# OpenNLPLab/ACR_WSSS

Measured on NVIDIA B200. Metric: train_imgs_per_sec, higher is better.
Workload: dtype bf16

## Files before the change

acr_wsss_b200/csrc/gelu.cu:

```cuda
#include "common.cuh"
#include <cuda_bf16.h>

namespace {

constexpr float kRsqrt2 = 0.70710678118654752440f;
constexpr float kRsqrt2Pi = 0.39894228040143267794f;
constexpr int kGeluChunks = 64;

__device__ __forceinline__ void phi_and_exp(float x, float& phi, float& e) {
  const float ax = fabsf(x);
  float t;
  asm("rcp.approx.ftz.f32 %0, %1;" : "=f"(t) : "f"(fmaf(0.3275911f * kRsqrt2, ax, 1.f)));
  asm("ex2.approx.ftz.f32 %0, %1;" : "=f"(e) : "f"(x * x * -0.72134752044448170368f));
  float p = 0.5f * 1.061405429f;
  p = fmaf(p, t, 0.5f * -1.453152027f);
  p = fmaf(p, t, 0.5f * 1.421413741f);
  p = fmaf(p, t, 0.5f * -0.284496736f);
  p = fmaf(p, t, 0.5f * 0.254829592f);
  const float h = p * t * e;
  phi = x < 0.f ? h : 1.f - h;
}
__device__ __forceinline__ float gelu_f(float x) {
  float phi, e;
  phi_and_exp(x, phi, e);
  return x * phi;
}
__device__ __forceinline__ float gelu_grad_f(float x) {
  float phi, e;
  phi_and_exp(x, phi, e);
  return fmaf(x * kRsqrt2Pi, e, phi);
}

__device__ __forceinline__ void unpack8(const uint4& v, float* f) {
  const __nv_bfloat162* h = reinterpret_cast<const __nv_bfloat162*>(&v);
#pragma unroll
  for (int i = 0; i < 4; ++i) {
    const float2 t = __bfloat1622float2(h[i]);
    f[2 * i] = t.x;
    f[2 * i + 1] = t.y;
  }
}
__device__ __forceinline__ uint4 pack8(const float* f) {
  uint4 v;
  __nv_bfloat162* h = reinterpret_cast<__nv_bfloat162*>(&v);
#pragma unroll
  for (int i = 0; i < 4; ++i) h[i] = __floats2bfloat162_rn(f[2 * i], f[2 * i + 1]);
  return v;
}

__global__ void __launch_bounds__(256)
gelu_fwd_kernel(const __nv_bfloat16* __restrict__ x, __nv_bfloat16* __restrict__ y, long long n) {
  const long long nv = n >> 3;
  const long long stride = (long long)gridDim.x * blockDim.x;
  for (long long i = (long long)blockIdx.x * blockDim.x + threadIdx.x; i < nv; i += stride) {
    const uint4 v = __ldg(reinterpret_cast<const uint4*>(x) + i);
    float f[8];
    unpack8(v, f);
#pragma unroll
    for (int e = 0; e < 8; ++e) f[e] = gelu_f(f[e]);
    reinterpret_cast<uint4*>(y)[i] = pack8(f);
  }
  if (blockIdx.x == 0 && threadIdx.x < (n & 7)) {
    const long long i = (nv << 3) + threadIdx.x;
    y[i] = __float2bfloat16(gelu_f(__bfloat162float(x[i])));
  }
}

__global__ void __launch_bounds__(256)
gelu_bwd_kernel(const __nv_bfloat16* __restrict__ x, const __nv_bfloat16* __restrict__ dy, __nv_bfloat16* __restrict__ dx,
                int M, int F, int rows_per_chunk, float* __restrict__ partial) {
  __shared__ float red[8][32][9];
  const int cg = threadIdx.x & 31, ty = threadIdx.x >> 5;
  const int c = blockIdx.x * 256 + cg * 8;
  const int r0 = blockIdx.y * rows_per_chunk;
  const int r1 = min(M, r0 + rows_per_chunk);
  float acc[8];
#pragma unroll
  for (int e = 0; e < 8; ++e) acc[e] = 0.f;
  if (c < F) {
#pragma unroll 2
    for (int r = r0 + ty; r < r1; r += 8) {
      const size_t off = ((size_t)r * F + c) >> 3;
      const uint4 xv = __ldg(reinterpret_cast<const uint4*>(x) + off);
      const uint4 gv = __ldg(reinterpret_cast<const uint4*>(dy) + off);
      float xf[8], gf[8];
      unpack8(xv, xf);
      unpack8(gv, gf);
#pragma unroll
      for (int e = 0; e < 8; ++e) gf[e] *= gelu_grad_f(xf[e]);
      const uint4 o = pack8(gf);
      reinterpret_cast<uint4*>(dx)[off] = o;
      unpack8(o, gf);
#pragma unroll
      for (int e = 0; e < 8; ++e) acc[e] += gf[e];
    }
  }
  if (partial == nullptr) return;
#pragma unroll
  for (int e = 0; e < 8; ++e) red[ty][cg][e] = acc[e];
  __syncthreads();
  const int col = threadIdx.x;
  if (blockIdx.x * 256 + col < F) {
    float t = 0.f;
#pragma unroll
    for (int k = 0; k < 8; ++k) t += red[k][col >> 3][col & 7];
    partial[(size_t)blockIdx.y * F + blockIdx.x * 256 + col] = t;
  }
}

__global__ void __launch_bounds__(256)
gelu_colsum_finish_kernel(const float* __restrict__ partial, int nparts, int F, float* __restrict__ out, int accumulate) {
  __shared__ float red[4][64];
  const int cl = threadIdx.x & 63, grp = threadIdx.x >> 6;
  const int c = blockIdx.x * 64 + cl;
  float s0 = 0.f, s1 = 0.f;
  if (c < F) {
    int p = grp;
    for (; p + 4 < nparts; p += 8) {
      s0 += __ldg(partial + (size_t)p * F + c);
      s1 += __ldg(partial + (size_t)(p + 4) * F + c);
    }
    for (; p < nparts; p += 4) s0 += __ldg(partial + (size_t)p * F + c);
  }
  red[grp][cl] = s0 + s1;
  __syncthreads();
  if (grp == 0 && c < F) {
    const float s = (red[0][cl] + red[1][cl]) + (red[2][cl] + red[3][cl]);
    out[c] = accumulate ? out[c] + s : s;
  }
}

}

extern "C" int acr_gelu_fwd_bf16(const void* x, void* y, long long n, void* stream) {
  ACR_REQUIRE(x && y, ACR_E_INVAL, "acr_gelu_fwd_bf16: null pointer");
  ACR_REQUIRE(n > 0, ACR_E_INVAL, "acr_gelu_fwd_bf16: n must be positive");
  ACR_REQUIRE((((uintptr_t)x | (uintptr_t)y) & 15) == 0, ACR_E_ALIGN, "acr_gelu_fwd_bf16: 16-byte alignment required");
  const long long nv = (n + 7) >> 3;
  const unsigned grid = (unsigned)std::min<long long>((nv + 255) / 256, 148LL * 32);
  gelu_fwd_kernel<<<grid, 256, 0, (cudaStream_t)stream>>>((const __nv_bfloat16*)x, (__nv_bfloat16*)y, n);
  return acr::check_launch("gelu_fwd_kernel");
}

extern "C" size_t acr_gelu_bwd_workspace(int F) { return F > 0 ? (size_t)kGeluChunks * F * sizeof(float) : 0; }

extern "C" int acr_gelu_bwd_bf16(const void* x, const void* dy, void* dx, int M, int F, float* colsum, int accumulate,
                                 void* workspace, size_t workspace_bytes, void* stream) {
  ACR_REQUIRE(x && dy && dx, ACR_E_INVAL, "acr_gelu_bwd_bf16: null pointer");
  ACR_REQUIRE(M > 0 && F > 0 && F % 8 == 0, ACR_E_INVAL, "acr_gelu_bwd_bf16: F must be a positive multiple of 8");
  ACR_REQUIRE((((uintptr_t)x | (uintptr_t)dy | (uintptr_t)dx) & 15) == 0, ACR_E_ALIGN, "acr_gelu_bwd_bf16: 16-byte alignment required");
  ACR_REQUIRE(colsum == nullptr || (workspace != nullptr && workspace_bytes >= acr_gelu_bwd_workspace(F)), ACR_E_NOMEM,
              "acr_gelu_bwd_bf16: workspace too small");
  cudaStream_t st = (cudaStream_t)stream;
  const int chunks = M < kGeluChunks * 8 ? 1 : kGeluChunks;
  const int rows_per_chunk = (M + chunks - 1) / chunks;
  dim3 grid((F + 255) / 256, chunks);
  gelu_bwd_kernel<<<grid, 256, 0, st>>>((const __nv_bfloat16*)x, (const __nv_bfloat16*)dy, (__nv_bfloat16*)dx, M, F, rows_per_chunk,
                                        colsum ? (float*)workspace : nullptr);
  if (int e = acr::check_launch("gelu_bwd_kernel")) return e;
  if (colsum) {
    gelu_colsum_finish_kernel<<<(F + 63) / 64, 256, 0, st>>>((const float*)workspace, chunks, F, colsum, accumulate);
    return acr::check_launch("gelu_colsum_finish_kernel");
  }
  return 0;
}
```

acr_wsss_b200/csrc/layernorm.cu:

```cuda
#include "attn_tc.cuh"
#include <cuda_bf16.h>

namespace {

constexpr int kWarpsPerCta = 8;

template <bool BF16>
__device__ __forceinline__ float4 load4(const void* __restrict__ base, long long idx4) {
  if (BF16) {
    const uint2 u = __ldg(reinterpret_cast<const uint2*>(base) + idx4);
    const float2 a = __bfloat1622float2(*reinterpret_cast<const __nv_bfloat162*>(&u.x));
    const float2 b = __bfloat1622float2(*reinterpret_cast<const __nv_bfloat162*>(&u.y));
    return make_float4(a.x, a.y, b.x, b.y);
  }
  return __ldg(reinterpret_cast<const float4*>(base) + idx4);
}
template <bool BF16>
__device__ __forceinline__ void store4(void* __restrict__ base, long long idx4, float4 v) {
  if (BF16) {
    __nv_bfloat162 p0 = __floats2bfloat162_rn(v.x, v.y), p1 = __floats2bfloat162_rn(v.z, v.w);
    uint2 u;
    u.x = *reinterpret_cast<uint32_t*>(&p0);
    u.y = *reinterpret_cast<uint32_t*>(&p1);
    reinterpret_cast<uint2*>(base)[idx4] = u;
  } else {
    reinterpret_cast<float4*>(base)[idx4] = v;
  }
}

template <int VEC, bool OUT_BF16, bool X_BF16>
__global__ void __launch_bounds__(kWarpsPerCta * 32)
layernorm_fwd_kernel(const void* __restrict__ x, const void* __restrict__ res, void* __restrict__ sum_out, const float* __restrict__ gamma,
                     const float* __restrict__ beta, int M, float eps, void* __restrict__ y, float* __restrict__ mean, float* __restrict__ rstd) {
  constexpr int E = 128 * VEC;
  const int lane = threadIdx.x & 31;
  for (long long row = (long long)blockIdx.x * kWarpsPerCta + (threadIdx.x >> 5); row < M; row += (long long)gridDim.x * kWarpsPerCta) {
  float4 v[VEC];
  float s = 0.f;
#pragma unroll
  for (int i = 0; i < VEC; ++i) {
    v[i] = load4<X_BF16>(x, row * (E / 4) + i * 32 + lane);
    if (res != nullptr) {
      const float4 r = load4<X_BF16>(res, row * (E / 4) + i * 32 + lane);
      v[i] = make_float4(v[i].x + r.x, v[i].y + r.y, v[i].z + r.z, v[i].w + r.w);
      if (X_BF16) {
        v[i].x = __bfloat162float(__float2bfloat16(v[i].x)); v[i].y = __bfloat162float(__float2bfloat16(v[i].y));
        v[i].z = __bfloat162float(__float2bfloat16(v[i].z)); v[i].w = __bfloat162float(__float2bfloat16(v[i].w));
      }
      store4<X_BF16>(sum_out, row * (E / 4) + i * 32 + lane, v[i]);
    }
    s += (v[i].x + v[i].y) + (v[i].z + v[i].w);
  }
  const float mu = acr::warp_sum(s) * (1.f / E);
  float ss = 0.f;
#pragma unroll
  for (int i = 0; i < VEC; ++i) {
    const float a = v[i].x - mu, b = v[i].y - mu, c = v[i].z - mu, d = v[i].w - mu;
    ss += (a * a + b * b) + (c * c + d * d);
  }
  const float rs = rsqrtf(acr::warp_sum(ss) * (1.f / E) + eps);
  if (lane == 0) { mean[row] = mu; rstd[row] = rs; }
#pragma unroll
  for (int i = 0; i < VEC; ++i) {
    const float4 g = __ldg(reinterpret_cast<const float4*>(gamma) + i * 32 + lane);
    const float4 bb = __ldg(reinterpret_cast<const float4*>(beta) + i * 32 + lane);
    const float o0 = (v[i].x - mu) * rs * g.x + bb.x, o1 = (v[i].y - mu) * rs * g.y + bb.y;
    const float o2 = (v[i].z - mu) * rs * g.z + bb.z, o3 = (v[i].w - mu) * rs * g.w + bb.w;
    store4<OUT_BF16>(y, row * (E / 4) + i * 32 + lane, make_float4(o0, o1, o2, o3));
  }
  }
}

template <int VEC, bool DY_BF16, bool X_BF16, bool COLSUM = false>
__global__ void __launch_bounds__(kWarpsPerCta * 32)
layernorm_bwd_kernel(const void* __restrict__ dy, const void* __restrict__ dres, const void* __restrict__ x, const float* __restrict__ mean,
                     const float* __restrict__ rstd, const float* __restrict__ gamma, int M, int rows_per_cta,
                     void* __restrict__ dx, float* __restrict__ part_g, float* __restrict__ part_b, float* __restrict__ part_c) {
  constexpr int E = 128 * VEC;
  constexpr int NARR = COLSUM ? 3 : 2;
  extern __shared__ float4 acc_sm[];
  const int lane = threadIdx.x & 31, warp = threadIdx.x >> 5;
  float4* ag = acc_sm + (0 * kWarpsPerCta + warp) * (VEC * 32) + lane;
  float4* ab = acc_sm + (1 * kWarpsPerCta + warp) * (VEC * 32) + lane;
  float4* ac = acc_sm + ((COLSUM ? 2 : 1) * kWarpsPerCta + warp) * (VEC * 32) + lane;
  float4 g[VEC];
#pragma unroll
  for (int i = 0; i < VEC; ++i) {
    g[i] = __ldg(reinterpret_cast<const float4*>(gamma) + i * 32 + lane);
    ag[i * 32] = make_float4(0.f, 0.f, 0.f, 0.f);
    ab[i * 32] = make_float4(0.f, 0.f, 0.f, 0.f);
    if (COLSUM) ac[i * 32] = make_float4(0.f, 0.f, 0.f, 0.f);
  }
  const long long r0 = (long long)blockIdx.x * rows_per_cta;
  const long long r1 = min((long long)M, r0 + rows_per_cta);
  for (long long row = r0 + warp; row < r1; row += kWarpsPerCta) {
    const float mu = __ldg(mean + row), rs = __ldg(rstd + row);
    float4 d[VEC], xh[VEC];
    float s1 = 0.f, s2 = 0.f;
#pragma unroll
    for (int i = 0; i < VEC; ++i) {
      d[i] = load4<DY_BF16>(dy, row * (E / 4) + i * 32 + lane);
      const float4 xv = load4<X_BF16>(x, row * (E / 4) + i * 32 + lane);
      xh[i] = make_float4((xv.x - mu) * rs, (xv.y - mu) * rs, (xv.z - mu) * rs, (xv.w - mu) * rs);
    }
#pragma unroll
    for (int i = 0; i < VEC; ++i) {
      float4 tb = ab[i * 32], tg = ag[i * 32];
      tb.x += d[i].x; tb.y += d[i].y; tb.z += d[i].z; tb.w += d[i].w;
      tg.x += d[i].x * xh[i].x; tg.y += d[i].y * xh[i].y; tg.z += d[i].z * xh[i].z; tg.w += d[i].w * xh[i].w;
      ab[i * 32] = tb;
      ag[i * 32] = tg;
      d[i].x *= g[i].x; d[i].y *= g[i].y; d[i].z *= g[i].z; d[i].w *= g[i].w;
      s1 += (d[i].x + d[i].y) + (d[i].z + d[i].w);
      s2 += (d[i].x * xh[i].x + d[i].y * xh[i].y) + (d[i].z * xh[i].z + d[i].w * xh[i].w);
    }
    s1 = acr::warp_sum(s1) * (1.f / E);
    s2 = acr::warp_sum(s2) * (1.f / E);
#pragma unroll
    for (int i = 0; i < VEC; ++i) {
      float4 o;
      o.x = rs * (d[i].x - s1 - xh[i].x * s2); o.y = rs * (d[i].y - s1 - xh[i].y * s2);
      o.z = rs * (d[i].z - s1 - xh[i].z * s2); o.w = rs * (d[i].w - s1 - xh[i].w * s2);
      if (dres != nullptr) {
        const float4 r = load4<X_BF16>(dres, row * (E / 4) + i * 32 + lane);
        o.x += r.x; o.y += r.y; o.z += r.z; o.w += r.w;
      }
      store4<X_BF16>(dx, row * (E / 4) + i * 32 + lane, o);
      if (COLSUM) {
        if (X_BF16) {
          o.x = __bfloat162float(__float2bfloat16(o.x)); o.y = __bfloat162float(__float2bfloat16(o.y));
          o.z = __bfloat162float(__float2bfloat16(o.z)); o.w = __bfloat162float(__float2bfloat16(o.w));
        }
        float4 tc_ = ac[i * 32];
        tc_.x += o.x; tc_.y += o.y; tc_.z += o.z; tc_.w += o.w;
        ac[i * 32] = tc_;
      }
    }
  }
  __syncthreads();
  const float* accf = reinterpret_cast<const float*>(acc_sm);
  for (int a = 0; a < NARR; ++a) {
    float* dst = (a == 0 ? part_g : (a == 1 ? part_b : part_c)) + (long long)blockIdx.x * E;
    for (int c = threadIdx.x; c < E; c += kWarpsPerCta * 32) {
      float t = 0.f;
#pragma unroll
      for (int w = 0; w < kWarpsPerCta; ++w) t += accf[(a * kWarpsPerCta + w) * E + c];
      dst[c] = t;
    }
  }
}

__global__ void __launch_bounds__(1024)
layernorm_bwd_finish_kernel(const float* __restrict__ part_g, const float* __restrict__ part_b, const float* __restrict__ part_c, int nparts,
                            int E, float* __restrict__ dgamma, float* __restrict__ dbeta, float* __restrict__ dx_colsum, int accumulate) {
  __shared__ float sg[128][9], sb[128][9], sc[128][9];
  const int cl = threadIdx.x & 7, grp = threadIdx.x >> 3;
  const int c = blockIdx.x * 8 + cl;
  float ag = 0.f, ab = 0.f, ac = 0.f;
  if (c < E) {
#pragma unroll 3
    for (int p = grp; p < nparts; p += 128) {
      ag += __ldg(part_g + (long long)p * E + c);
      ab += __ldg(part_b + (long long)p * E + c);
      if (part_c != nullptr) ac += __ldg(part_c + (long long)p * E + c);
    }
  }
  sg[grp][cl] = ag;
  sb[grp][cl] = ab;
  sc[grp][cl] = ac;
  __syncthreads();
  if (threadIdx.x < 24 && blockIdx.x * 8 + (threadIdx.x & 7) < E) {
    const int arr = threadIdx.x >> 3, col = threadIdx.x & 7;
    const float (*src)[9] = arr == 0 ? sg : (arr == 1 ? sb : sc);
    float t0 = 0.f, t1 = 0.f, t2 = 0.f, t3 = 0.f;
#pragma unroll 8
    for (int k = 0; k < 128; k += 4) { t0 += src[k][col]; t1 += src[k + 1][col]; t2 += src[k + 2][col]; t3 += src[k + 3][col]; }
    const float t = (t0 + t1) + (t2 + t3);
    const int cc = blockIdx.x * 8 + col;
    if (arr == 0) dgamma[cc] = accumulate ? dgamma[cc] + t : t;
    else if (arr == 1) dbeta[cc] = accumulate ? dbeta[cc] + t : t;
    else if (dx_colsum != nullptr) dx_colsum[cc] = accumulate ? dx_colsum[cc] + t : t;
  }
}

constexpr int kColsumChunks = 64;

__global__ void __launch_bounds__(256)
colsum_bf16_kernel(const __nv_bfloat16* __restrict__ x, int M, int F, int rows_per_chunk, float* __restrict__ partial) {
  __shared__ float2 red[8][33];
  const int cp = threadIdx.x & 31, grp = threadIdx.x >> 5;
  const int c = blockIdx.x * 64 + cp * 2;
  const int r0 = blockIdx.y * rows_per_chunk;
  const int r1 = min(M, r0 + rows_per_chunk);
  float2 acc = make_float2(0.f, 0.f);
  if (c < F) {
    for (int r = r0 + grp; r < r1; r += 8) {
      const float2 v = __bfloat1622float2(*reinterpret_cast<const __nv_bfloat162*>(x + (size_t)r * F + c));
      acc.x += v.x;
      acc.y += v.y;
    }
  }
  red[grp][cp] = acc;
  __syncthreads();
  if (grp == 0 && c < F) {
    float2 t = make_float2(0.f, 0.f);
#pragma unroll
    for (int k = 0; k < 8; ++k) { t.x += red[k][cp].x; t.y += red[k][cp].y; }
    *reinterpret_cast<float2*>(partial + (size_t)blockIdx.y * F + c) = t;
  }
}

__global__ void __launch_bounds__(256)
colsum_finish_kernel(const float* __restrict__ partial, int nparts, int F, float* __restrict__ out, int accumulate) {
  __shared__ float red[4][64];
  const int cl = threadIdx.x & 63, grp = threadIdx.x >> 6;
  const int c = blockIdx.x * 64 + cl;
  float s0 = 0.f, s1 = 0.f;
  if (c < F) {
    int p = grp;
    for (; p + 4 < nparts; p += 8) {
      s0 += __ldg(partial + (size_t)p * F + c);
      s1 += __ldg(partial + (size_t)(p + 4) * F + c);
    }
    for (; p < nparts; p += 4) s0 += __ldg(partial + (size_t)p * F + c);
  }
  red[grp][cl] = s0 + s1;
  __syncthreads();
  if (grp == 0 && c < F) {
    const float s = (red[0][cl] + red[1][cl]) + (red[2][cl] + red[3][cl]);
    out[c] = accumulate ? out[c] + s : s;
  }
}

constexpr int kBwdCtas = 296;

template <int VEC>
int launch_fwd(const void* x, int x_bf16, const void* res, void* sum_out, const float* gamma, const float* beta, int M, float eps, void* y, int y_bf16, float* mean,
               float* rstd, cudaStream_t st) {
  const unsigned grid = (unsigned)std::min((M + kWarpsPerCta - 1) / kWarpsPerCta, 148 * 8);
  const int T = kWarpsPerCta * 32;
  if (x_bf16) {
    if (y_bf16) layernorm_fwd_kernel<VEC, true, true><<<grid, T, 0, st>>>(x, res, sum_out, gamma, beta, M, eps, y, mean, rstd);
    else layernorm_fwd_kernel<VEC, false, true><<<grid, T, 0, st>>>(x, res, sum_out, gamma, beta, M, eps, y, mean, rstd);
  } else {
    if (y_bf16) layernorm_fwd_kernel<VEC, true, false><<<grid, T, 0, st>>>(x, res, sum_out, gamma, beta, M, eps, y, mean, rstd);
    else layernorm_fwd_kernel<VEC, false, false><<<grid, T, 0, st>>>(x, res, sum_out, gamma, beta, M, eps, y, mean, rstd);
  }
  return acr::check_launch("layernorm_fwd_kernel");
}
template <int VEC>
int launch_bwd(const void* dy, int dy_bf16, const void* dres, const void* x, int x_bf16, const float* mean, const float* rstd, const float* gamma, int M,
               void* dx, float* dgamma, float* dbeta, float* dx_colsum, int accumulate, float* parts, cudaStream_t st) {
  constexpr int E = 128 * VEC;
  const int ctas = M < kBwdCtas * kWarpsPerCta ? (M + kWarpsPerCta - 1) / kWarpsPerCta : kBwdCtas;
  const int rows_per_cta = (M + ctas - 1) / ctas;
  float* pg = parts;
  float* pb = parts + (size_t)kBwdCtas * E;
  float* pc = dx_colsum ? parts + (size_t)2 * kBwdCtas * E : nullptr;
  const int T = kWarpsPerCta * 32;
#define ACR_LN_BWD(DYB, XB, CS)                                                                                              \
  do {                                                                                                                      \
    auto kfn = layernorm_bwd_kernel<VEC, DYB, XB, CS>;                                                                      \
    const size_t smem = (size_t)(CS ? 3 : 2) * kWarpsPerCta * E * sizeof(float);                                            \
    static bool attr_set[64] = {false};             \
    if (int e_ = acr_attn::set_max_smem(kfn, smem, attr_set)) return e_;                                                    \
    kfn<<<ctas, T, smem, st>>>(dy, dres, x, mean, rstd, gamma, M, rows_per_cta, dx, pg, pb, pc);                            \
  } while (0)
  if (pc != nullptr) {
    ACR_REQUIRE(x_bf16 && dy_bf16, ACR_E_INVAL, "acr_layernorm_bwd: dx_colsum needs bf16 x and dy");
    ACR_LN_BWD(true, true, true);
  } else if (x_bf16) {
    if (dy_bf16) ACR_LN_BWD(true, true, false);
    else ACR_LN_BWD(false, true, false);
  } else {
    if (dy_bf16) ACR_LN_BWD(true, false, false);
    else ACR_LN_BWD(false, false, false);
  }
#undef ACR_LN_BWD
  if (int e = acr::check_launch("layernorm_bwd_kernel")) return e;
  layernorm_bwd_finish_kernel<<<(E + 7) / 8, 1024, 0, st>>>(pg, pb, pc, ctas, E, dgamma, dbeta, dx_colsum, accumulate);
  return acr::check_launch("layernorm_bwd_finish_kernel");
}

}

extern "C" size_t acr_layernorm_bwd_workspace(int E) { return E > 0 ? (size_t)3 * kBwdCtas * E * sizeof(float) : 0; }

extern "C" int acr_layernorm_fwd(const void* x, int x_is_bf16, const void* residual, void* sum_out, const float* gamma, const float* beta,
                                 int M, int E, float eps, void* y, int y_is_bf16, float* mean, float* rstd, void* stream) {
  ACR_REQUIRE(x && gamma && beta && y && mean && rstd, ACR_E_INVAL, "acr_layernorm_fwd: null pointer");
  ACR_REQUIRE(M > 0 && E > 0 && E % 128 == 0 && E <= 2048, ACR_E_INVAL, "acr_layernorm_fwd: E=%d must be a multiple of 128, <= 2048", E);
  ACR_REQUIRE((residual == nullptr) == (sum_out == nullptr), ACR_E_INVAL, "acr_layernorm_fwd: residual and sum_out go together");
  ACR_REQUIRE((((uintptr_t)x | (uintptr_t)y | (uintptr_t)gamma | (uintptr_t)beta | (uintptr_t)residual | (uintptr_t)sum_out) & 15) == 0, ACR_E_ALIGN,
              "acr_layernorm_fwd: 16-byte alignment required");
  cudaStream_t st = (cudaStream_t)stream;
  switch (E / 128) {
    case 1: return launch_fwd<1>(x, x_is_bf16, residual, sum_out, gamma, beta, M, eps, y, y_is_bf16, mean, rstd, st);
    case 2: return launch_fwd<2>(x, x_is_bf16, residual, sum_out, gamma, beta, M, eps, y, y_is_bf16, mean, rstd, st);
    case 3: return launch_fwd<3>(x, x_is_bf16, residual, sum_out, gamma, beta, M, eps, y, y_is_bf16, mean, rstd, st);
    case 4: return launch_fwd<4>(x, x_is_bf16, residual, sum_out, gamma, beta, M, eps, y, y_is_bf16, mean, rstd, st);
    case 6: return launch_fwd<6>(x, x_is_bf16, residual, sum_out, gamma, beta, M, eps, y, y_is_bf16, mean, rstd, st);
    case 8: return launch_fwd<8>(x, x_is_bf16, residual, sum_out, gamma, beta, M, eps, y, y_is_bf16, mean, rstd, st);
    case 10: return launch_fwd<10>(x, x_is_bf16, residual, sum_out, gamma, beta, M, eps, y, y_is_bf16, mean, rstd, st);
    case 12: return launch_fwd<12>(x, x_is_bf16, residual, sum_out, gamma, beta, M, eps, y, y_is_bf16, mean, rstd, st);
    case 16: return launch_fwd<16>(x, x_is_bf16, residual, sum_out, gamma, beta, M, eps, y, y_is_bf16, mean, rstd, st);
    default: acr::set_error("acr_layernorm_fwd: E=%d unsupported (128*{1,2,3,4,6,8,10,12,16})", E); return ACR_E_INVAL;
  }
}

extern "C" int acr_layernorm_bwd(const void* dy, int dy_is_bf16, const void* d_residual, const void* x, int x_is_bf16, const float* mean, const float* rstd,
                                 const float* gamma, int M, int E, void* dx, float* dgamma, float* dbeta, float* dx_colsum, int accumulate,
                                 void* workspace, size_t workspace_bytes, void* stream) {
  ACR_REQUIRE(dy && x && mean && rstd && gamma && dx && dgamma && dbeta && workspace, ACR_E_INVAL, "acr_layernorm_bwd: null pointer");
  ACR_REQUIRE(M > 0 && E > 0 && E % 128 == 0 && E <= 2048, ACR_E_INVAL, "acr_layernorm_bwd: E=%d must be a multiple of 128, <= 2048", E);
  ACR_REQUIRE(workspace_bytes >= acr_layernorm_bwd_workspace(E), ACR_E_NOMEM, "acr_layernorm_bwd: workspace too small");
  ACR_REQUIRE((((uintptr_t)x | (uintptr_t)dy | (uintptr_t)dx | (uintptr_t)gamma | (uintptr_t)workspace | (uintptr_t)d_residual) & 15) == 0, ACR_E_ALIGN,
              "acr_layernorm_bwd: 16-byte alignment required");
  cudaStream_t st = (cudaStream_t)stream;
  float* parts = (float*)workspace;
  switch (E / 128) {
    case 1: return launch_bwd<1>(dy, dy_is_bf16, d_residual, x, x_is_bf16, mean, rstd, gamma, M, dx, dgamma, dbeta, dx_colsum, accumulate, parts, st);
    case 2: return launch_bwd<2>(dy, dy_is_bf16, d_residual, x, x_is_bf16, mean, rstd, gamma, M, dx, dgamma, dbeta, dx_colsum, accumulate, parts, st);
    case 3: return launch_bwd<3>(dy, dy_is_bf16, d_residual, x, x_is_bf16, mean, rstd, gamma, M, dx, dgamma, dbeta, dx_colsum, accumulate, parts, st);
    case 4: return launch_bwd<4>(dy, dy_is_bf16, d_residual, x, x_is_bf16, mean, rstd, gamma, M, dx, dgamma, dbeta, dx_colsum, accumulate, parts, st);
    case 6: return launch_bwd<6>(dy, dy_is_bf16, d_residual, x, x_is_bf16, mean, rstd, gamma, M, dx, dgamma, dbeta, dx_colsum, accumulate, parts, st);
    case 8: return launch_bwd<8>(dy, dy_is_bf16, d_residual, x, x_is_bf16, mean, rstd, gamma, M, dx, dgamma, dbeta, dx_colsum, accumulate, parts, st);
    case 10: return launch_bwd<10>(dy, dy_is_bf16, d_residual, x, x_is_bf16, mean, rstd, gamma, M, dx, dgamma, dbeta, dx_colsum, accumulate, parts, st);
    case 12: return launch_bwd<12>(dy, dy_is_bf16, d_residual, x, x_is_bf16, mean, rstd, gamma, M, dx, dgamma, dbeta, dx_colsum, accumulate, parts, st);
    case 16: return launch_bwd<16>(dy, dy_is_bf16, d_residual, x, x_is_bf16, mean, rstd, gamma, M, dx, dgamma, dbeta, dx_colsum, accumulate, parts, st);
    default: acr::set_error("acr_layernorm_bwd: E=%d unsupported (128*{1,2,3,4,6,8,10,12,16})", E); return ACR_E_INVAL;
  }
}

extern "C" size_t acr_colsum_workspace(int F) { return F > 0 ? (size_t)kColsumChunks * F * sizeof(float) : 0; }

extern "C" int acr_colsum_bf16(const void* x, int M, int F, float* out, int accumulate, void* workspace, size_t workspace_bytes,
                               void* stream) {
  ACR_REQUIRE(x && out && workspace, ACR_E_INVAL, "acr_colsum_bf16: null pointer");
  ACR_REQUIRE(M > 0 && F > 0 && F % 2 == 0, ACR_E_INVAL, "acr_colsum_bf16: F must be even");
  ACR_REQUIRE(workspace_bytes >= acr_colsum_workspace(F), ACR_E_NOMEM, "acr_colsum_bf16: workspace too small");
  ACR_REQUIRE(((uintptr_t)x & 3) == 0 && ((uintptr_t)workspace & 7) == 0, ACR_E_ALIGN, "acr_colsum_bf16: alignment");
  cudaStream_t st = (cudaStream_t)stream;
  const int chunks = M < kColsumChunks * 8 ? 1 : kColsumChunks;
  const int rows_per_chunk = (M + chunks - 1) / chunks;
  dim3 grid((F + 63) / 64, chunks);
  colsum_bf16_kernel<<<grid, 256, 0, st>>>((const __nv_bfloat16*)x, M, F, rows_per_chunk, (float*)workspace);
  if (int e = acr::check_launch("colsum_bf16_kernel")) return e;
  colsum_finish_kernel<<<(F + 63) / 64, 256, 0, st>>>((const float*)workspace, chunks, F, out, accumulate);
  return acr::check_launch("colsum_finish_kernel");
}
```

Baseline: 578.6.

## Prefetch rows in layernorm bwd, vectorize colsum, one-row-per-warp LN fwd

The layernorm backward loads the next row's dy, x and residual into registers one step ahead, when they fit a register budget. It also reads gamma from cache per element instead of keeping it in registers, and adds a min-blocks launch bound to raise occupancy. The layernorm forward drops the grid-stride loop and launches one warp per row. Column-sum reads 8 bf16 per 128-bit load when aligned, and several loops get larger unroll pragmas. These target memory latency and bandwidth in small elementwise and reduction kernels, at the cost of more register pressure and a larger forward grid.

```diff
diff --git a/acr_wsss_b200/csrc/gelu.cu b/acr_wsss_b200/csrc/gelu.cu
--- a/acr_wsss_b200/csrc/gelu.cu
+++ b/acr_wsss_b200/csrc/gelu.cu
@@ -78,7 +78,7 @@
 #pragma unroll
   for (int e = 0; e < 8; ++e) acc[e] = 0.f;
   if (c < F) {
-#pragma unroll 2
+#pragma unroll 4
     for (int r = r0 + ty; r < r1; r += 8) {
       const size_t off = ((size_t)r * F + c) >> 3;
       const uint4 xv = __ldg(reinterpret_cast<const uint4*>(x) + off);
@@ -116,6 +116,7 @@
   float s0 = 0.f, s1 = 0.f;
   if (c < F) {
     int p = grp;
+#pragma unroll 8
     for (; p + 4 < nparts; p += 8) {
       s0 += __ldg(partial + (size_t)p * F + c);
       s1 += __ldg(partial + (size_t)(p + 4) * F + c);
diff --git a/acr_wsss_b200/csrc/layernorm.cu b/acr_wsss_b200/csrc/layernorm.cu
--- a/acr_wsss_b200/csrc/layernorm.cu
+++ b/acr_wsss_b200/csrc/layernorm.cu
@@ -1,19 +1,26 @@
 #include "attn_tc.cuh"
 #include <cuda_bf16.h>
+#include <type_traits>
 
 namespace {
 
 constexpr int kWarpsPerCta = 8;
 
+template <bool BF16> struct Raw4 { using T = float4; };
+template <> struct Raw4<true> { using T = uint2; };
+template <bool BF16>
+__device__ __forceinline__ typename Raw4<BF16>::T load_raw4(const void* __restrict__ base, long long idx4) {
+  return __ldg(reinterpret_cast<const typename Raw4<BF16>::T*>(base) + idx4);
+}
+__device__ __forceinline__ float4 widen4(float4 v) { return v; }
+__device__ __forceinline__ float4 widen4(uint2 u) {
+  const float2 a = __bfloat1622float2(*reinterpret_cast<const __nv_bfloat162*>(&u.x));
+  const float2 b = __bfloat1622float2(*reinterpret_cast<const __nv_bfloat162*>(&u.y));
+  return make_float4(a.x, a.y, b.x, b.y);
+}
 template <bool BF16>
 __device__ __forceinline__ float4 load4(const void* __restrict__ base, long long idx4) {
-  if (BF16) {
-    const uint2 u = __ldg(reinterpret_cast<const uint2*>(base) + idx4);
-    const float2 a = __bfloat1622float2(*reinterpret_cast<const __nv_bfloat162*>(&u.x));
-    const float2 b = __bfloat1622float2(*reinterpret_cast<const __nv_bfloat162*>(&u.y));
-    return make_float4(a.x, a.y, b.x, b.y);
-  }
-  return __ldg(reinterpret_cast<const float4*>(base) + idx4);
+  return widen4(load_raw4<BF16>(base, idx4));
 }
 template <bool BF16>
 __device__ __forceinline__ void store4(void* __restrict__ base, long long idx4, float4 v) {
@@ -34,7 +41,8 @@
                      const float* __restrict__ beta, int M, float eps, void* __restrict__ y, float* __restrict__ mean, float* __restrict__ rstd) {
   constexpr int E = 128 * VEC;
   const int lane = threadIdx.x & 31;
-  for (long long row = (long long)blockIdx.x * kWarpsPerCta + (threadIdx.x >> 5); row < M; row += (long long)gridDim.x * kWarpsPerCta) {
+  const long long row = (long long)blockIdx.x * kWarpsPerCta + (threadIdx.x >> 5);
+  if (row >= M) return;
   float4 v[VEC];
   float s = 0.f;
 #pragma unroll
@@ -68,11 +76,10 @@
     const float o2 = (v[i].z - mu) * rs * g.z + bb.z, o3 = (v[i].w - mu) * rs * g.w + bb.w;
     store4<OUT_BF16>(y, row * (E / 4) + i * 32 + lane, make_float4(o0, o1, o2, o3));
   }
-  }
 }
 
 template <int VEC, bool DY_BF16, bool X_BF16, bool COLSUM = false>
-__global__ void __launch_bounds__(kWarpsPerCta * 32)
+__global__ void __launch_bounds__(kWarpsPerCta * 32, VEC <= 8 ? 2 : 1)
 layernorm_bwd_kernel(const void* __restrict__ dy, const void* __restrict__ dres, const void* __restrict__ x, const float* __restrict__ mean,
                      const float* __restrict__ rstd, const float* __restrict__ gamma, int M, int rows_per_cta,
                      void* __restrict__ dx, float* __restrict__ part_g, float* __restrict__ part_b, float* __restrict__ part_c) {
@@ -83,46 +90,70 @@
   float4* ag = acc_sm + (0 * kWarpsPerCta + warp) * (VEC * 32) + lane;
   float4* ab = acc_sm + (1 * kWarpsPerCta + warp) * (VEC * 32) + lane;
   float4* ac = acc_sm + ((COLSUM ? 2 : 1) * kWarpsPerCta + warp) * (VEC * 32) + lane;
-  float4 g[VEC];
 #pragma unroll
   for (int i = 0; i < VEC; ++i) {
-    g[i] = __ldg(reinterpret_cast<const float4*>(gamma) + i * 32 + lane);
     ag[i * 32] = make_float4(0.f, 0.f, 0.f, 0.f);
     ab[i * 32] = make_float4(0.f, 0.f, 0.f, 0.f);
     if (COLSUM) ac[i * 32] = make_float4(0.f, 0.f, 0.f, 0.f);
   }
+  const float4* gamma4 = reinterpret_cast<const float4*>(gamma) + lane;
   const long long r0 = (long long)blockIdx.x * rows_per_cta;
   const long long r1 = min((long long)M, r0 + rows_per_cta);
+  using RawDy = typename Raw4<DY_BF16>::T;
+  using RawX = typename Raw4<X_BF16>::T;
+  constexpr bool kAhead = VEC * (sizeof(RawDy) + 2 * sizeof(RawX)) <= 36 * 4;
+  RawDy dy_n[VEC];
+  RawX x_n[VEC], dr_n[VEC];
+  float mu_n = 0.f, rs_n = 0.f;
+  auto fetch = [&](long long row) {
+    if (row >= r1) return;
+    mu_n = __ldg(mean + row);
+    rs_n = __ldg(rstd + row);
+#pragma unroll
+    for (int i = 0; i < VEC; ++i) {
+      dy_n[i] = load_raw4<DY_BF16>(dy, row * (E / 4) + i * 32 + lane);
+      x_n[i] = load_raw4<X_BF16>(x, row * (E / 4) + i * 32 + lane);
+      if (dres != nullptr) dr_n[i] = load_raw4<X_BF16>(dres, row * (E / 4) + i * 32 + lane);
+    }
+  };
+  if (kAhead) fetch(r0 + warp);
   for (long long row = r0 + warp; row < r1; row += kWarpsPerCta) {
-    const float mu = __ldg(mean + row), rs = __ldg(rstd + row);
-    float4 d[VEC], xh[VEC];
+    if (!kAhead) fetch(row);
+    const float mu = mu_n, rs = rs_n;
+    RawDy dyr[VEC];
+    RawX xr[VEC], dr[VEC];
+#pragma unroll
+    for (int i = 0; i < VEC; ++i) { dyr[i] = dy_n[i]; xr[i] = x_n[i]; dr[i] = dr_n[i]; }
+    if (kAhead) fetch(row + kWarpsPerCta);
+    auto xhat = [&](int i) {
+      const float4 xv = widen4(xr[i]);
+      return make_float4((xv.x - mu) * rs, (xv.y - mu) * rs, (xv.z - mu) * rs, (xv.w - mu) * rs);
+    };
+    float4 dg[VEC];
     float s1 = 0.f, s2 = 0.f;
 #pragma unroll
     for (int i = 0; i < VEC; ++i) {
-      d[i] = load4<DY_BF16>(dy, row * (E / 4) + i * 32 + lane);
-      const float4 xv = load4<X_BF16>(x, row * (E / 4) + i * 32 + lane);
-      xh[i] = make_float4((xv.x - mu) * rs, (xv.y - mu) * rs, (xv.z - mu) * rs, (xv.w - mu) * rs);
-    }
-#pragma unroll
-    for (int i = 0; i < VEC; ++i) {
+      const float4 d = widen4(dyr[i]), xh = xhat(i);
       float4 tb = ab[i * 32], tg = ag[i * 32];
-      tb.x += d[i].x; tb.y += d[i].y; tb.z += d[i].z; tb.w += d[i].w;
-      tg.x += d[i].x * xh[i].x; tg.y += d[i].y * xh[i].y; tg.z += d[i].z * xh[i].z; tg.w += d[i].w * xh[i].w;
+      tb.x += d.x; tb.y += d.y; tb.z += d.z; tb.w += d.w;
+      tg.x += d.x * xh.x; tg.y += d.y * xh.y; tg.z += d.z * xh.z; tg.w += d.w * xh.w;
       ab[i * 32] = tb;
       ag[i * 32] = tg;
-      d[i].x *= g[i].x; d[i].y *= g[i].y; d[i].z *= g[i].z; d[i].w *= g[i].w;
-      s1 += (d[i].x + d[i].y) + (d[i].z + d[i].w);
-      s2 += (d[i].x * xh[i].x + d[i].y * xh[i].y) + (d[i].z * xh[i].z + d[i].w * xh[i].w);
+      const float4 g = __ldg(gamma4 + i * 32);
+      dg[i] = make_float4(d.x * g.x, d.y * g.y, d.z * g.z, d.w * g.w);
+      s1 += (dg[i].x + dg[i].y) + (dg[i].z + dg[i].w);
+      s2 += (dg[i].x * xh.x + dg[i].y * xh.y) + (dg[i].z * xh.z + dg[i].w * xh.w);
     }
     s1 = acr::warp_sum(s1) * (1.f / E);
     s2 = acr::warp_sum(s2) * (1.f / E);
 #pragma unroll
     for (int i = 0; i < VEC; ++i) {
+      const float4 xh = xhat(i);
       float4 o;
-      o.x = rs * (d[i].x - s1 - xh[i].x * s2); o.y = rs * (d[i].y - s1 - xh[i].y * s2);
-      o.z = rs * (d[i].z - s1 - xh[i].z * s2); o.w = rs * (d[i].w - s1 - xh[i].w * s2);
+      o.x = rs * (dg[i].x - s1 - xh.x * s2); o.y = rs * (dg[i].y - s1 - xh.y * s2);
+      o.z = rs * (dg[i].z - s1 - xh.z * s2); o.w = rs * (dg[i].w - s1 - xh.w * s2);
       if (dres != nullptr) {
-        const float4 r = load4<X_BF16>(dres, row * (E / 4) + i * 32 + lane);
+        const float4 r = widen4(dr[i]);
         o.x += r.x; o.y += r.y; o.z += r.z; o.w += r.w;
       }
       store4<X_BF16>(dx, row * (E / 4) + i * 32 + lane, o);
@@ -185,28 +216,41 @@
 
 constexpr int kColsumChunks = 64;
 
-__global__ void __launch_bounds__(256)
+template <int V>
+__global__ void __launch_bounds__(256, 4)
 colsum_bf16_kernel(const __nv_bfloat16* __restrict__ x, int M, int F, int rows_per_chunk, float* __restrict__ partial) {
-  __shared__ float2 red[8][33];
-  const int cp = threadIdx.x & 31, grp = threadIdx.x >> 5;
-  const int c = blockIdx.x * 64 + cp * 2;
+  using Vec = typename std::conditional<V == 8, uint4, uint32_t>::type;
+  static_assert(sizeof(Vec) == 2 * V, "V bf16 per load");
+  __shared__ float red[8][32][V + 1];
+  const int cg = threadIdx.x & 31, grp = threadIdx.x >> 5;
+  const int c = blockIdx.x * 32 * V + cg * V;
   const int r0 = blockIdx.y * rows_per_chunk;
   const int r1 = min(M, r0 + rows_per_chunk);
-  float2 acc = make_float2(0.f, 0.f);
+  float acc[V];
+#pragma unroll
+  for (int e = 0; e < V; ++e) acc[e] = 0.f;
   if (c < F) {
+#pragma unroll 4
     for (int r = r0 + grp; r < r1; r += 8) {
-      const float2 v = __bfloat1622float2(*reinterpret_cast<const __nv_bfloat162*>(x + (size_t)r * F + c));
-      acc.x += v.x;
-      acc.y += v.y;
-    }
-  }
-  red[grp][cp] = acc;
+      const Vec u = __ldg(reinterpret_cast<const Vec*>(x + (size_t)r * F + c));
+      const __nv_bfloat162* h = reinterpret_cast<const __nv_bfloat162*>(&u);
+#pragma unroll
+      for (int e = 0; e < V / 2; ++e) {
+        const float2 v = __bfloat1622float2(h[e]);
+        acc[2 * e] += v.x;
+        acc[2 * e + 1] += v.y;
+      }
+    }
+  }
+#pragma unroll
+  for (int e = 0; e < V; ++e) red[grp][cg][e] = acc[e];
   __syncthreads();
-  if (grp == 0 && c < F) {
-    float2 t = make_float2(0.f, 0.f);
-#pragma unroll
-    for (int k = 0; k < 8; ++k) { t.x += red[k][cp].x; t.y += red[k][cp].y; }
-    *reinterpret_cast<float2*>(partial + (size_t)blockIdx.y * F + c) = t;
+  for (int col = threadIdx.x; col < 32 * V; col += 256) {
+    if (blockIdx.x * 32 * V + col >= F) break;
+    float t = 0.f;
+#pragma unroll
+    for (int k = 0; k < 8; ++k) t += red[k][col / V][col % V];
+    partial[(size_t)blockIdx.y * F + blockIdx.x * 32 * V + col] = t;
   }
 }
 
@@ -218,6 +262,7 @@
   float s0 = 0.f, s1 = 0.f;
   if (c < F) {
     int p = grp;
+#pragma unroll 8
     for (; p + 4 < nparts; p += 8) {
       s0 += __ldg(partial + (size_t)p * F + c);
       s1 += __ldg(partial + (size_t)(p + 4) * F + c);
@@ -237,7 +282,7 @@
 template <int VEC>
 int launch_fwd(const void* x, int x_bf16, const void* res, void* sum_out, const float* gamma, const float* beta, int M, float eps, void* y, int y_bf16, float* mean,
                float* rstd, cudaStream_t st) {
-  const unsigned grid = (unsigned)std::min((M + kWarpsPerCta - 1) / kWarpsPerCta, 148 * 8);
+  const unsigned grid = (unsigned)((M + kWarpsPerCta - 1) / kWarpsPerCta);
   const int T = kWarpsPerCta * 32;
   if (x_bf16) {
     if (y_bf16) layernorm_fwd_kernel<VEC, true, true><<<grid, T, 0, st>>>(x, res, sum_out, gamma, beta, M, eps, y, mean, rstd);
@@ -343,8 +388,10 @@
   cudaStream_t st = (cudaStream_t)stream;
   const int chunks = M < kColsumChunks * 8 ? 1 : kColsumChunks;
   const int rows_per_chunk = (M + chunks - 1) / chunks;
-  dim3 grid((F + 63) / 64, chunks);
-  colsum_bf16_kernel<<<grid, 256, 0, st>>>((const __nv_bfloat16*)x, M, F, rows_per_chunk, (float*)workspace);
+  if (F % 8 == 0 && ((uintptr_t)x & 15) == 0)
+    colsum_bf16_kernel<8><<<dim3((F + 255) / 256, chunks), 256, 0, st>>>((const __nv_bfloat16*)x, M, F, rows_per_chunk, (float*)workspace);
+  else
+    colsum_bf16_kernel<2><<<dim3((F + 63) / 64, chunks), 256, 0, st>>>((const __nv_bfloat16*)x, M, F, rows_per_chunk, (float*)workspace);
   if (int e = acr::check_launch("colsum_bf16_kernel")) return e;
   colsum_finish_kernel<<<(F + 63) / 64, 256, 0, st>>>((const float*)workspace, chunks, F, out, accumulate);
   return acr::check_launch("colsum_finish_kernel");
```

Result: no change. 578.2 (median of 6 runs) (-0.1%).
